# xubiker/deephisto

Measured on AMD Instinct MI355X. Metric: 256x256 patches/sec WSI inference (predict_full_patched), higher is better.
Workload: dtype bf16; 1 GPU; BASELINE configs[2]: predict_full_patched on one 50000x50000x3 closed-form synthetic WSI resident in HBM, 256x256 tiles stride 256, ResNet-18 (random init), bf16 MFMA, step = one whole slide (tile grid -> fused gather+forward -> all-gather -> ordered accumulate -> argmax); patch=256, stride=256, sampler_batch=64, micro_batch=4096, streams=1, downscale=16, n_tiles=38416, n_classes=5, parallelism=tile-range shard x1

## Files before the change

### deephisto_amd/_lib.py

```python
from __future__ import annotations

import ctypes as C
from pathlib import Path

import torch

LIB_PATH = Path(__file__).resolve().parent / "libdeephisto_hip.so"

DH_LAYOUT_NHWC, DH_LAYOUT_NCHW = 0, 1
DH_DTYPE_F32, DH_DTYPE_BF16 = 0, 1

_i32, _i64, _u32 = C.c_int32, C.c_int64, C.c_uint32
BUCKET_CB = C.CFUNCTYPE(None, C.c_int32, C.c_int64, C.c_int64, C.c_void_p)
_p = C.c_void_p

SIGNATURES = {
    "dh_abi_version": (C.c_int, []),
    "dh_last_error": (C.c_char_p, []),
    "dh_tile_grid_count": (C.c_int, [_i64, _i64, _i32, _i32, _i32, C.POINTER(_i64), C.POINTER(_i64)]),
    "dh_tile_grid": (C.c_int, [_i64, _i64, _i32, _i32, _i32, _p, _i64]),
    "dh_synth_slide": (C.c_int, [_p, _i64, _i64, _u32, _p]),
    "dh_tile_gather": (C.c_int, [_p, _i64, _i64, _p, _p, _i64, _i32, _i32, _i32, _p, _p]),
    "dh_tile_gather_aug": (C.c_int, [_p, _i64, _i64, _p, _i64, _i32, _i32, _i32, _i32, _i32, _p, _p]),
    "dh_tile_gather_stain_aug": (C.c_int, [_p, _i64, _i64, _p, _p, _p, _i64, _i32, _i32, _i32, _i32, _i32, _p, _p, _i32, _p, _i32, _p, _p]),
# ... 114 lines not shown
    "dh_debug_wgrad_bf16": (C.c_int, [_p, _p, _p] + [_i32] * 8 + [_p]),
    "dh_debug_conv_bf16": (C.c_int, [_p, _p, _p, _p] + [_i32] * 8 + [_p]),
    "dh_debug_conv_bn_act":(C.c_int, [_p, _p, _p, _p, _p, _p] + [_i32] * 9 + [_p]),
    "dh_debug_stem_out": (C.c_int, [_p, _i64, _i32, _p, _p]),
    "dh_debug_stem_pool_bf16": (C.c_int, [_p, _p, _i64, _i64, _p, _i64, _i32, _p, _p]),
    "dh_debug_wgrad_f32": (C.c_int, [_p, _p, _p] + [_i32] * 8 + [_p]),
    "dh_debug_stem_wgrad_f32": (C.c_int, [_p, _p, _p, _i32, _i32, _p]),
    "dh_debug_dgrad_f32": (C.c_int, [_p, _p, _p, _p] + [_i32] * 7 + [_p]),
    "dh_debug_pack_f32": (C.c_int, [_p, _i32, _i32, _p, _p, _p, _p, _p]),
    "dh_debug_pack_bf16": (C.c_int, [_p, _i32, _i32, _p, _p, _p, _p, _p]),
    "dh_debug_bn_f32": (C.c_int, [_p, _p, _p, _p, _i32, _p, _p, _p, _p, _p, _p, _p, _i64, _i32, _p]),
    "dh_debug_maxpool_f32": (C.c_int, [_p, _p, _p, _p, _i32, _i32, _i32, _i32, _p]),
    "dh_debug_bn_pool_f32": (C.c_int, [_p, _p, _p, _p, _p, _p, _p, _p, _p, _i32, _i32, _i32, _i32, _p]),
    "dh_debug_stamps": (C.c_int, [_i32, _p]),
    "dh_debug_stem_strip_width": (C.c_int, [_i32]),
    "dh_debug_last_conv3": (C.c_int, [_p, _p]),
    "dh_debug_env_knobs": (C.c_int, [C.c_char_p, _i64]),
    "dh_debug_coverage_set_map": (C.c_int, [_p, _p, _p]),
    "dh_debug_resnet18_forward_tap": (C.c_int, [_p, _p, _i64, _i64, _p, _i64, _i32, C.c_char_p, _p, _i32, _p, _i64, _p, _p]),
    "dh_debug_resnet50_forward_tap": (C.c_int, [_p, _p, _i64, _i64, _p, _i64, _i32, C.c_char_p, _p, _i32, _p, _i64, _p, _p]),
    "dh_debug_resnet18_operands": (C.c_int, [_p, C.c_char_p, _p, _i64, _p, _p, _i64]),
    "dh_debug_resnet50_operands": (C.c_int, [_p, C.c_char_p, _p, _i64, _p, _p, _i64]),
}


class DeephistoHipError(RuntimeError):
    pass


_lib = None
# ... 22 lines not shown
```

### deephisto_amd/csrc/conv3_tables_host.h

```cpp
#pragma once
#include <algorithm>
#include <array>
#include <cstdint>
#include <map>
#include <vector>

namespace dh_conv3 {

constexpr int kChunkBytes = 64;

struct TileDesc { int x, y, z, w; };

struct HostTables {
  std::vector<int> lane;
  std::vector<TileDesc> tile;
  std::vector<unsigned> mask;
  int grid = 0, threads = 0, lane_stride = 0, mask_rows = 0;
  bool xcd_group = false;
};

template <int STRIDE, int NT, int WAVES>
constexpr int max_window_pieces() { return (STRIDE == 2) ? (WAVES == 8 ? 5 : 10) : (NT == 2 ? 6 : 4); }

struct Cand { int th, tw, imgs, hp, variant, hr = 0, wtail = 0, fit = 0, ip = 0; };
// ... 154 lines not shown
inline int m16_read_conflicts(const int (&bl)[64]) {
  int extra = 0;
  for (int sg = 0; sg < 4; ++sg) {
    int cnt[16] = {0};
    for (int ll = 0; ll < 32; ++ll) {
      const bool in_a = ll < 4 || (ll >= 12 && ll < 16) || (ll >= 20 && ll < 28);
      if (in_a != ((sg & 1) == 0)) continue;
      const int l = (sg >> 1) * 32 + ll, G = l >> 4, slot = ((G & 1) << 1) | (G >> 1), w = bl[l];
      ++cnt[((w & 3) << 2) | (slot ^ ((w >> 2) & 3))];
    }
    for (int b = 0; b < 16; ++b) extra += cnt[b] > 1 ? cnt[b] - 1 : 0;
  }
  return extra;
}

template <int STRIDE, int NT, int WAVES, int ESZ, int MT, class P, bool HALF = false, bool M16 = false>
const char* build_tables(const P& p, int ncb, int grid_override, HostTables* out) {
  static_assert(!M16 || (STRIDE == 1 && !HALF && ESZ == 2), "M16: the stride-1 bf16 kernels");
  constexpr int MAXJ = max_window_pieces<STRIDE, NT, WAVES>();
  constexpr int NB = M16 ? 2 * NT : NT;
  const int threads = WAVES * 64, stride = 2 * NT + NB + MAXJ;
  constexpr int STAGE_PX_BYTES = HALF ? kChunkBytes / 2 : kChunkBytes;
  if ((int64_t)p.Cin * ESZ < 2 * STAGE_PX_BYTES || ((int64_t)p.Cin * ESZ) % STAGE_PX_BYTES) return "conv3x3: needs at least two whole channel stages per tile";
  const int64_t win_px = (int64_t)p.IMGS * p.HR * p.HP + p.WTAIL;
  const int IP = p.IP ? p.IP : p.HR * p.HP;
  if (win_px * STAGE_PX_BYTES > 65536) return "conv3x3: staged window larger than 64 KiB (16-bit fragment offsets)";
  if ((int64_t)p.n_win_instr * 1024 < win_px * STAGE_PX_BYTES) return "conv3x3: the DMA plan does not cover the staged window";
  constexpr int NTILE32 = (HALF ? WAVES / 2 : WAVES * MT / 2) * NT;
  if (p.FIT) {
    if (STRIDE != 1 || HALF) return "conv3x3: fit tiles are stride-1 tiles";
    if (p.IMGS * p.TH * p.TW > NTILE32 * 32) return "conv3x3: fit tile larger than the workgroup's slots";
    if (p.HP < p.TW + 1 || p.HR < p.TH + 1) return "conv3x3: fit tile pitch too small";
// ... 85 lines not shown
      for (int j = 0; j < MAXJ; ++j) {
        const auto& w = win[(size_t)tid * MAXJ + j];
        const int iy = oy0 * STRIDE + w[0] - 1, ix = ox0 * STRIDE + w[1] - 1;
        if (w[3] && w[2] < mk[2] && iy >= 0 && iy < p.Hi && ix >= 0 && ix < p.Wi) m |= 1u << j;
      }
      for (int nt = 0; nt < NT; ++nt) {
        const auto& q = pix[(size_t)tid * NT + nt];
        if (q[2] < mk[2] && oy0 + q[0] < p.Ho && ox0 + q[1] < p.Wo) m |= 1u << (16 + nt);
      }
      mask[(size_t)r * threads + tid] = m;
    }
    return r;
  };
  const int tiles_per_img = p.tiles_y * p.tiles_x;
  const int grid = grid_override > 0 ? grid_override : std::min(256, p.ntiles), n_pt = p.ntiles / ncb;
  const bool xcd_group = ncb > 1 && grid == 256 && 32 % ncb == 0 && (int64_t)p.Cout * p.Cin * 9 * ESZ <= (1 << 23);
  std::vector<TileDesc>& tile = out->tile;
  tile.assign((size_t)p.iters * grid, TileDesc{0, 0, 0, 0});
  for (int it = 0; it < p.iters; ++it)
    for (int w = 0; w < grid; ++w) {
      int cb, pt;
      if (xcd_group) {
        const int xcd = w % 8, slot = w / 8;
        cb = slot % ncb;
        pt = it * (grid / ncb) + (slot / ncb) * 8 + xcd;
      } else {
        const int T_ = it * grid + w;
        cb = T_ % ncb; pt = T_ / ncb;
      }
      const int valid = pt < n_pt ? 1 : 0, t = pt % tiles_per_img;
      const int img0 = valid ? (pt / tiles_per_img) * p.IMGS : 0, oy0 = (t / p.tiles_x) * p.TH, ox0 = (t % p.tiles_x) * p.TW;
      const int mrow = mask_row_of(img0, oy0, ox0);
      if (mrow >= 4096) return "conv3x3: too many distinct tile positions for the mask table";
      const int64_t win_off = (int64_t)img0 * img_in_bytes + ((int64_t)(oy0 * STRIDE) * p.Wi + ox0 * STRIDE) * p.in_px_bytes;
      const int64_t out_off = (int64_t)img0 * p.o_img + (int64_t)oy0 * p.o_row + (int64_t)ox0 * p.o_px + p.o_base + (int64_t)cb * p.out_cb;
      const int64_t res_off = (int64_t)img0 * p.o_img + (int64_t)oy0 * p.r_row + (int64_t)ox0 * p.r_px + p.r_base + (int64_t)cb * p.r_cb;
      if (win_off >= ((int64_t)1 << 32) || out_off >= ((int64_t)1 << 32) || res_off >= ((int64_t)1 << 32)) return "conv3x3: tensor larger than 4 Gi elements / bytes";
      const uint32_t word = (uint32_t)cb | (uint32_t)valid << 16 | (uint32_t)mrow << 20;
      tile[(size_t)it * grid + w] = TileDesc{(int)word, (int)(uint32_t)win_off, (int)(uint32_t)out_off, (int)(uint32_t)res_off};
    }
  out->grid = grid; out->threads = threads; out->lane_stride = stride; out->mask_rows = (int)mask_row.size(); out->xcd_group = xcd_group;
  return nullptr;
}

}
// ... 1 lines not shown
```

### deephisto_amd/csrc/env_knobs.h

```cpp
#pragma once

#define DH_ENV_KNOBS(X)                                                                                                                  \
  X(DH_CONV_S2_WIDE, 1, 0, 1, "load", "bf16 inference: 1 = wide stride-2 + downsample kernel (128 couts x 256 pixels), 0 = 128-pixel kernel")      \
  X(DH_CONV_FIT, 1, 0, 1, "load", "3x3 stride-1 convs on 7x7 / 14x14 maps: 1 = fit tiles (ten 7x7 images / five 7x14 half-images per 512 slots), 0 = power-of-two tiles")   \
  X(DH_CONV_MFMA16, 1, 0, 1, "load", "bf16 3x3 stride-1 convs: 1 = 16x16x32 MFMAs on the layers where they measured faster, 0 = 32x32x16 everywhere")   \
  X(DH_T1_SIDE, 1, 0, 1, "create", "float32 training engine: weight gradients on a low-priority side stream")                                     \
  X(DH_WGRAD3_WGS, 0, 0, 256, "load", "float32 3x3 weight gradient: workgroups per launch (0 = 224 with the side stream, else 256)")              \
  X(DH_T2_SIDE, 1, 0, 1, "create", "bf16 training engine: weight gradients, Adam and re-pack on a low-priority side stream")                       \
  X(DH_T2_JOIN, 1, 0, 1, "create", "bf16 engine: downsample branch's BN applied inside the join BN's pass (bit-identical either way)")            \
  X(DH_T2_FOLD, 1, 0, 1, "create", "bf16 engine: BN finalize folded into channel-sliced consumers on small maps (bit-identical either way)")      \
  X(DH_T2_FOLD_ROWS, 16384, 0, 1 << 24, "load", "bf16 engine: largest map (rows = B*H*W) that takes the folded BN path")                          \
  X(DH_G2_NSTAGE, 0, 0, 3, "load", "bf16 1x1 GEMM: LDS ring depth (0 = automatic: 2, or 3 from K >= DH_G2_NS3_K)")                                 \
  X(DH_G2_NS3_K, 512, 64, 1 << 20, "load", "bf16 1x1 GEMM: K from which the ring runs three stages deep")                                          \
  X(DH_G2_WIDE_M, 0, 0, 1 << 30, "load", "bf16 1x1 GEMM: 128 x 128 tiles for GEMMs of up to this many pixels (0 = off)")                          \
  X(DH_WGRAD_RING, 1, 0, 1, "load", "bf16 1x1 weight gradient: LDS-DMA ring kernel (0 = round-3 register-staged kernel)")                          \
  X(DH_WGRAD_RING_WGS, 0, 0, 1024, "load", "bf16 ring weight gradient: workgroups per launch (0 = 128 with the side stream, else 256)")           \
  X(DH_WGRAD2_WGS, 0, 0, 256, "load", "bf16 3x3 / 64-channel weight gradient: workgroups per launch (0 = 224 with the side stream, else 256)")
```

### deephisto_amd/csrc/resnet50_infer.inc

```

constexpr int R50_MAX_P = 256;
constexpr int64_t R50_MAX_TILES = ((int64_t)1 << 31) / ((int64_t)256 * (R50_MAX_P / 4) * (R50_MAX_P / 4) * 2);
static_assert(R50_MAX_TILES == DH_RESNET50_MAX_TILES, "include/deephisto_hip.h states the launch limit");

struct dh_resnet50 : InferNet {
  float* ones = nullptr;
  std::vector<int32_t> yx_host;
};

namespace {

struct R50GemmCfg { int nmt, nstage; };
R50GemmCfg r50_gemm_cfg(int N, int K) {
  R50GemmCfg c;
  c.nmt = (N % 128 == 0 && K <= 1024) ? 4 : 2;
  c.nstage = std::min(K / G2_BK, 2);
  return c;
}

int r50_gemm(const ConvLayer& L, const bf16_t* in, const bf16_t* res, bf16_t* out, int B, int Hi, int Wi, bool relu, hipStream_t st) {
  const int Ho = (Hi - 1) / L.stride + 1, Wo = (Wi - 1) / L.stride + 1;
  const int64_t M = (int64_t)B * Ho * Wo;
  DH_REQUIRE(L.ks == 1 && L.cout % 64 == 0 && L.cin % 64 == 0 && M > 0 && M < ((int64_t)1 << 31),
             "resnet50 1x1 %s: M=%lld N=%d K=%d unsupported", L.name.c_str(), (long long)M, L.cout, L.cin);
// ... 22 lines not shown
  auto al = [](size_t v) { return (v + 255) & ~(size_t)255; };
  const size_t px = (size_t)B * H2 * H2 * 2;
  const size_t big = al(256 * px), t1 = al(128 * px), t2 = al(64 * px);
  const size_t need = 2 * big + t1 + t2;
  int rc;
  if ((rc = infer_workspace(net, need))) return rc;
  char* base = static_cast<char*>(net->ws);
  bf16_t* X = reinterpret_cast<bf16_t*>(base);
  bf16_t* D = reinterpret_cast<bf16_t*>(base + big);
  bf16_t* T1 = reinterpret_cast<bf16_t*>(base + 2 * big);
  bf16_t* T2 = reinterpret_cast<bf16_t*>(base + 2 * big + t1);
  DH_REQUIRE(stem_seam_bytes(B, P) <= t1, "resnet50 forward: seam scratch larger than the bottleneck buffer");
  if ((rc = launch_stem_pool(net->convs[0], x, slide, slide_h, slide_w, yx, B, P, X, T1, st))) return rc;
  for (const char* nm : {"conv1", "maxpool"})
    if ((rc = tap_after<__bf16>(tap, nm, X, 64, H2, H2, 32, st))) return rc;
  int H = H2;
  for (const BlockDesc& b : net->desc->blocks) {
    const ConvLayer &c1 = net->convs[b.conv[0]], &c2 = net->convs[b.conv[1]], &c3 = net->convs[b.conv[2]];
    const int Ho = (H - 1) / b.stride + 1;
    if ((rc = r50_gemm(c1, X, nullptr, T1, B, H, H, true, st))) return rc;
    if ((rc = tap_after<__bf16>(tap, c1.name, T1, c1.cout, H, H, 32, st))) return rc;
    rc = b.stride == 1 ? launch_conv3x3<__bf16, 1>(c2, T1, nullptr, T2, B, H, H, true, st, Ho, Ho, nullptr, nullptr, true)
                       : launch_conv3x3<__bf16, 2>(c2, T1, nullptr, T2, B, H, H, true, st, Ho, Ho, nullptr, nullptr, true);
    if (rc) return rc;
    if ((rc = tap_after<__bf16>(tap, c2.name, T2, c2.cout, Ho, Ho, 32, st))) return rc;
    const bf16_t* idt = X;
    if (b.ds >= 0) {
      if ((rc = r50_gemm(net->convs[b.ds], X, nullptr, D, B, H, H, false, st))) return rc;
      if ((rc = tap_after<__bf16>(tap, net->convs[b.ds].name, D, c3.cout, Ho, Ho, 32, st))) return rc;
      idt = D;
    }
    if ((rc = r50_gemm(c3, T2, idt, X, B, Ho, Ho, true, st))) return rc;
    if ((rc = tap_after<__bf16>(tap, c3.name, X, c3.cout, Ho, Ho, 32, st))) return rc;
    H = Ho;
  }
  if (feat)
    hipLaunchKernelGGL(r50_head_kernel<true>, dim3(B), dim3(256), 0, st, X, H * H, net->fc_w_dev, net->fc_b_dev, net->n_classes, logits, feat);
  else if (logits)
// ... 133 lines not shown
```

### deephisto_amd/csrc/resnet_kernels.hip

```cpp
#include <math.h>
#include <stdlib.h>
#include <string.h>

#include <algorithm>
#include <array>
#include <atomic>
#include <map>
#include <mutex>
#include <set>
#include <string>
#include <vector>

#include "dh_common.h"
#include "conv3_tables_host.h"

typedef float f32x16 __attribute__((ext_vector_type(16)));
typedef float f32x4 __attribute__((ext_vector_type(4)));
typedef __bf16 bf16x8 __attribute__((ext_vector_type(8)));

namespace {

constexpr int CHUNK_BYTES = 64;
constexpr int PIX_PITCH = 80;
constexpr int FRAG_BYTES = 1024;
// ... 631 lines not shown
  if (it == g_zero_page.end()) {
    void* z = nullptr;
    DH_HIP(hipMalloc(&z, 1024));
    DH_HIP(hipMemset(z, 0, 1024));
    it = g_zero_page.emplace(dev, z).first;
  }
  *out = it->second;
  return DH_OK;
}

struct Conv3Tables { int* lane = nullptr; int4* tile = nullptr; unsigned* mask = nullptr; };
std::map<std::vector<int>, Conv3Tables> g_conv3_tables;
constexpr size_t CONV3_TABLE_CAP = 256;

template <int STRIDE, int NT, int WAVES, int ESZ, int MT, bool HALF = false, bool M16 = false>
int conv3_tables(const Conv3Params& p, int ncb, int groups_img, Conv3Tables* out, int grid_override = 0) {
  const std::vector<int> key = {current_device(), STRIDE, NT, WAVES, MT + (HALF ? 100 : 0) + (M16 ? 200 : 0), ESZ, p.TH, p.TW, p.IMGS, p.HR, p.HC, p.HP, p.HPH, p.Hi, p.Wi,
                                p.Cin, p.B, p.tiles_y, p.tiles_x, ncb, p.n_win_instr, p.WTAIL, p.FIT, p.IP, p.in_px_bytes, p.Ho, p.Wo, p.Cout, p.out_px,
                                p.out_cb, (int)(p.o_img & 0x7FFFFFFF), (int)(p.o_img >> 31), p.o_row, p.o_px, p.o_base, grid_override, p.iters,
                                p.r_row, p.r_px, p.r_cb, p.r_base};
  std::lock_guard<std::mutex> lk(g_host_mu);
  auto it = g_conv3_tables.find(key);
  if (it != g_conv3_tables.end()) { *out = it->second; return DH_OK; }
  if (g_conv3_tables.size() >= CONV3_TABLE_CAP) {
    for (auto& kv : g_conv3_tables) { (void)hipFree(kv.second.lane); (void)hipFree(kv.second.tile); (void)hipFree(kv.second.mask); }
    g_conv3_tables.clear();
  }
  dh_conv3::HostTables ht;
  if (const char* why = dh_conv3::build_tables<STRIDE, NT, WAVES, ESZ, MT, Conv3Params, HALF, M16>(p, ncb, grid_override, &ht)) { dh::set_error("%s", why); return DH_EINVAL; }
  static_assert(sizeof(dh_conv3::TileDesc) == sizeof(int4), "tile descriptor = int4");
  const std::vector<int>& lane = ht.lane;
  const std::vector<dh_conv3::TileDesc>& tile = ht.tile;
  const std::vector<unsigned>& mask = ht.mask;
  Conv3Tables tb;
  DH_HIP(hipMalloc((void**)&tb.lane, lane.size() * sizeof(int)));
  DH_HIP(hipMalloc((void**)&tb.tile, tile.size() * sizeof(int4)));
  DH_HIP(hipMalloc((void**)&tb.mask, mask.size() * sizeof(unsigned)));
  DH_HIP(hipMemcpy(tb.lane, lane.data(), lane.size() * sizeof(int), hipMemcpyHostToDevice));
  DH_HIP(hipMemcpy(tb.tile, tile.data(), tile.size() * sizeof(int4), hipMemcpyHostToDevice));
  DH_HIP(hipMemcpy(tb.mask, mask.data(), mask.size() * sizeof(unsigned), hipMemcpyHostToDevice));
  g_conv3_tables[key] = tb;
  *out = tb;
  (void)groups_img;
  return DH_OK;
}

template <typename T, int STRIDE, int NT, int WAVES, bool DS = false, int MT = 2, bool WRES = false, int CLS = -1, bool HALF = false, bool M16 = false>
int launch_conv3x3_cfg(Conv3Params& p, const ConvLayer& L, hipStream_t st) {
  constexpr int STAGE_PX_BYTES = HALF ? CHUNK_BYTES / 2 : CHUNK_BYTES, CO_BLK = HALF ? 128 : 64;
  const int win_px = p.IMGS * p.HR * p.HP + p.WTAIL;
  const int win_bytes = win_px * STAGE_PX_BYTES;
  const size_t wslab = (size_t)(9 + (DS ? 1 : 0)) * SLAB_TAP, win_alloc = (win_bytes + 1023) & ~1023;
  const size_t nchunks = (size_t)L.cin * sizeof(T) / STAGE_PX_BYTES;
  const size_t lds = (WRES ? nchunks * wslab + 2 * win_alloc : 2 * (wslab + win_alloc)) + (HALF ? 4096 : DS ? 2048 : 1024);

  constexpr int MAXJ = (STRIDE == 2) ? (WAVES == 8 ? 5 : 10) : (NT == 2 ? 6 : 4);
  p.n_win_instr = HALF ? (win_px + 31) / 32 : (win_px + 15) / 16;
  DH_REQUIRE(p.n_win_instr <= MAXJ * WAVES, "conv3x3: staging window too large for the DMA plan");
  DH_REQUIRE(lds <= 160 * 1024, "conv3x3: LDS budget exceeded (%zu B)", lds);
  DH_REQUIRE(p.FIT ? p.IMGS * p.TH * p.TW <= (WAVES * MT / 2) * NT * 32 && STRIDE == 1 && !HALF
                   : p.IMGS * p.TH * p.TW == (HALF ? WAVES / 2 : WAVES * MT / 2) * NT * 32, "conv3x3: tile/pixel mismatch");
  DH_REQUIRE(L.cin * (int)sizeof(T) >= 2 * CHUNK_BYTES, "conv3x3: needs at least two channel chunks");
  const int groups = ((p.B + p.IMGS - 1) / p.IMGS) * p.tiles_y * p.tiles_x;
  p.ntiles = groups * (L.cout / CO_BLK);
  const int grid = std::min(256, p.ntiles);
  DH_REQUIRE(!WRES || grid % (L.cout / 64) == 0, "conv3x3: resident weights need a fixed cout block per workgroup");
  p.iters = (p.ntiles + grid - 1) / grid;
  Conv3Tables tb;
  int rc = conv3_tables<STRIDE, NT, WAVES, (int)sizeof(T), MT, HALF, M16>(p, L.cout / CO_BLK, groups, &tb);
  if (rc) return rc;
  p.lane_tab = tb.lane; p.tile_tab = tb.tile; p.mask_tab = tb.mask;
  if constexpr (CLS >= 0) {
    if ((rc = ensure_dyn_lds(reinterpret_cast<const void*>(&conv3x3_kernel<T, STRIDE, NT, WAVES, false, DS, MT, WRES, CLS>), 160 * 1024))) return rc;
    hipLaunchKernelGGL((conv3x3_kernel<T, STRIDE, NT, WAVES, false, DS, MT, WRES, CLS>), dim3(grid), dim3(WAVES * 64), lds, st, p);
    DH_LAUNCH_CHECK();
    return DH_OK;
  }
  if ((rc = ensure_dyn_lds(reinterpret_cast<const void*>(&conv3x3_kernel<T, STRIDE, NT, WAVES, false, DS, MT, WRES, -1, HALF, M16>), 160 * 1024)) ||
      (rc = ensure_dyn_lds(reinterpret_cast<const void*>(&conv3x3_kernel<T, STRIDE, NT, WAVES, true, DS, MT, WRES, -1, HALF, M16>), 160 * 1024))) return rc;
  if (p.stamps) hipLaunchKernelGGL((conv3x3_kernel<T, STRIDE, NT, WAVES, true, DS, MT, WRES, -1, HALF, M16>), dim3(grid), dim3(WAVES * 64), lds, st, p);
  else hipLaunchKernelGGL((conv3x3_kernel<T, STRIDE, NT, WAVES, false, DS, MT, WRES, -1, HALF, M16>), dim3(grid), dim3(WAVES * 64), lds, st, p);
  DH_LAUNCH_CHECK();
  return DH_OK;
}

inline bool s2_wide_eligible(const ConvLayer& c1, const ConvLayer& ds, int esz, int Wo) {
  static const bool on = dh::env_int("DH_CONV_S2_WIDE") != 0;
  return on && esz == 2 && c1.w2_dev && ds.w2_dev && c1.cout % 128 == 0 && Wo > 4;
}

inline bool conv3_mfma16_layer(int cin, int cout) {
  static const bool on = dh::env_int("DH_CONV_MFMA16") != 0;
  return DH_CONV_HOIST && on && cin == cout && (cin == 64 || cin == 256 || cin == 512);
}
std::atomic<int> g_last_conv3_variant{-1}, g_last_conv3_mfma{0};

template <typename T, int STRIDE, int CLS = -1>
int launch_conv3x3(const ConvLayer& L, const void* in, const void* res, void* out, int B, int Hi, int Wi,
                   bool relu, hipStream_t st, int Ho, int Wo, const ConvLayer* ds = nullptr, void* ds_out = nullptr,
                   bool blocked = false, int full_h = 0, int full_w = 0, bool in16 = false, bool out16 = false) {
  Conv3Params p;
  static_assert(CLS < 0 || STRIDE == 1, "parity classes run on the stride-1 kernel");
  DH_REQUIRE(blocked || (!in16 && !out16), "conv3x3: 16-channel planes are a variant of the channel-blocked layout");
  DH_REQUIRE(CLS < 0 || (!blocked && !ds && full_h > 0 && full_w > 0), "conv3x3: a parity class needs the NHWC layout and the size of dX");
  DH_REQUIRE(!blocked || sizeof(T) == 2, "conv3x3: the channel-blocked layout is the bf16 inference layout");
  if (blocked) {
    p.in_px_bytes = CHUNK_BYTES; p.in_chunk_bytes = Hi * Wi * CHUNK_BYTES;
    p.out_px = 32; p.out_mt = Ho * Wo * 32; p.out_cb = 2 * p.out_mt;
  } else {
    p.in_px_bytes = L.cin * (int)sizeof(T); p.in_chunk_bytes = CHUNK_BYTES;
    p.out_px = L.cout; p.out_mt = 32; p.out_cb = 64;
  }
  if (CLS >= 0) {
    p.o_img = (int64_t)full_h * full_w * L.cout; p.o_row = 2 * full_w * L.cout; p.o_px = 2 * L.cout;
    p.o_base = ((CLS >> 1) * full_w + (CLS & 1)) * L.cout;
  } else {
// ... 43 lines not shown
    g_last_conv3_variant = -1; g_last_conv3_mfma = 32;
    if constexpr (CLS >= 0)
      rc = variant == 0 ? launch_conv3x3_cfg<T, 1, 2, 8, false, 2, false, CLS>(p, L, st)
         : variant == 1 ? launch_conv3x3_cfg<T, 1, 1, 8, false, 2, false, CLS>(p, L, st)
                        : launch_conv3x3_cfg<T, 1, 1, 8, false, 1, false, CLS>(p, L, st);
    else {
      constexpr bool BF16 = sizeof(T) == 2;
      const bool wres = BF16 && variant == 0 && wres_lds <= 160 * 1024;
      bool m16 = false;
#if DH_CONV_HOIST
      if constexpr (BF16) m16 = conv3_mfma16_layer(L.cin, L.cout);
#endif
      g_last_conv3_variant = variant; g_last_conv3_mfma = m16 ? 16 : 32;
      if constexpr (BF16 && DH_CONV_HOIST) {
        if (m16)
          rc = wres         ? launch_conv3x3_cfg<T, 1, 2, 8, false, 2, true, -1, false, true>(p, L, st)
             : variant == 0 ? launch_conv3x3_cfg<T, 1, 2, 8, false, 2, false, -1, false, true>(p, L, st)
             : variant == 1 ? launch_conv3x3_cfg<T, 1, 1, 8, false, 2, false, -1, false, true>(p, L, st)
                            : launch_conv3x3_cfg<T, 1, 1, 8, false, 1, false, -1, false, true>(p, L, st);
      }
      if (!m16)
        rc = wres         ? launch_conv3x3_cfg<T, 1, 2, 8, false, 2, BF16>(p, L, st)
           : variant == 0 ? launch_conv3x3_cfg<T, 1, 2, 8>(p, L, st)
           : variant == 1 ? launch_conv3x3_cfg<T, 1, 1, 8>(p, L, st)
                          : launch_conv3x3_cfg<T, 1, 1, 8, false, 1>(p, L, st);
    }
  } else {
    g_last_conv3_variant = -1; g_last_conv3_mfma = 32;
    static const bool s2_wide = dh::env_int("DH_CONV_S2_WIDE") != 0;
    if constexpr (sizeof(T) == 2) {
      if (in16) {
        DH_REQUIRE(s2_wide && ds && blocked && L.w2_dev && ds->w2_dev && L.cout % 128 == 0 && dh_conv3::set_stride2_wide_geometry(p, Ho, Wo),
                   "conv3x3: an input in 16-channel planes needs the wide stride-2 kernel");
        p.w = L.w2_dev; p.ds_w = ds->w2_dev;
        p.out_cb = 4 * p.out_mt;
        return launch_conv3x3_cfg<T, 2, 2, 8, true, 2, false, -1, true>(p, L, st);
      }
    }
    dh_conv3::set_stride2_geometry(p, Ho, Wo);
    const size_t wres_lds = (size_t)L.cin * sizeof(T) / CHUNK_BYTES * (ds ? 10 : 9) * SLAB_TAP
                          + 2 * (((size_t)p.IMGS * p.HR * p.HP * CHUNK_BYTES + 1023) & ~(size_t)1023) + 2048;
    if (ds && sizeof(T) == 2 && wres_lds <= 160 * 1024) rc = launch_conv3x3_cfg<T, 2, 1, 8, true, 1, true>(p, L, st);
    else rc = ds ? launch_conv3x3_cfg<T, 2, 1, 8, true, 1>(p, L, st) : launch_conv3x3_cfg<T, 2, 1, 8, false, 1>(p, L, st);
  }
  if (rc) return rc;
  if (sample) {
    DH_HIP(hipEventRecord(g_prof.ev[g_prof.used + 1], st));
    g_prof.used += 2;
    g_prof.flops += 2.0 * B * Ho * Wo * (double)L.cout * 9 * L.cin;
  }
  return DH_OK;
}

template <typename T, int NT, int WAVES, int MT>
int launch_dgrad_s2_merged_cfg(Conv3Params (&pc)[4], const int (&tiles_c)[4], const ConvLayer& L, hipStream_t st) {
  static const int order[4] = {3, 1, 2, 0}, taps[4] = {4, 2, 2, 1};
  constexpr int MAXJ = NT == 2 ? 6 : 4;
  const Conv3Params& p0 = pc[0];
// ... 110 lines not shown
    p.in = dz; p.w = L.w_dev; p.scale = L.scale_dev; p.shift = L.shift_dev; p.res = res; p.out = dx;
    p.B = B; p.Hi = Ho; p.Wi = Wo; p.Cin = L.cin; p.Cout = L.cout; p.Ho = rows; p.Wo = cols;
    p.relu = 0; p.zero_page = zp; p.stamps = nullptr;
    p.HPH = 0; p.TH = cd.th; p.TW = cd.tw; p.IMGS = cd.imgs; p.HP = cd.hp; p.HR = cd.th + 2; p.HC = cd.tw + 2;
    p.tiles_y = (rows + cd.th - 1) / cd.th; p.tiles_x = (cols + cd.tw - 1) / cd.tw;
    p.lane_tab = nullptr; p.tile_tab = nullptr; p.mask_tab = nullptr; p.ntiles = 0; p.iters = 0; p.n_win_instr = 0;
    tiles_c[k] = tiles_of(cd, rows, cols);
  }
  return cd.variant == 0 ? launch_dgrad_s2_merged_cfg<T, 2, 8, 2>(pc, tiles_c, L, st)
       : cd.variant == 1 ? launch_dgrad_s2_merged_cfg<T, 1, 8, 2>(pc, tiles_c, L, st)
                         : launch_dgrad_s2_merged_cfg<T, 1, 8, 1>(pc, tiles_c, L, st);
}

template <typename T>
int run_conv(const ConvLayer& L, const void* in, const void* res, void* out, int B, int Hi, int Wi,
             bool relu, hipStream_t st, int* Ho_out, int* Wo_out, bool blocked = false, bool out16 = false) {
  const int pad = L.ks / 2;
  const int Ho = (Hi + 2 * pad - L.ks) / L.stride + 1, Wo = (Wi + 2 * pad - L.ks) / L.stride + 1;
  *Ho_out = Ho; *Wo_out = Wo;
  DH_REQUIRE((int64_t)B * Hi * Wi * L.cin * (int64_t)sizeof(T) < ((int64_t)1 << 32),
             "conv %s: input larger than 4 GiB, reduce the batch", L.name.c_str());
  if (L.ks == 3 && L.stride == 1) return launch_conv3x3<T, 1>(L, in, res, out, B, Hi, Wi, relu, st, Ho, Wo, nullptr, nullptr, blocked, 0, 0, false, out16);
  DH_REQUIRE(!out16, "conv %s: only the stride-1 3x3 kernel writes 16-channel planes", L.name.c_str());
  if (L.ks == 3 && L.stride == 2) return launch_conv3x3<T, 2>(L, in, res, out, B, Hi, Wi, relu, st, Ho, Wo, nullptr, nullptr, blocked);
  DH_REQUIRE(!blocked, "conv %s: only the 3x3 kernels read the channel-blocked layout", L.name.c_str());
  ConvParams p;
  p.in = in; p.w = L.w_dev; p.scale = L.scale_dev; p.shift = L.shift_dev; p.res = res; p.out = out;
  p.B = B; p.Hi = Hi; p.Wi = Wi; p.Cin = L.cin; p.Cout = L.cout; p.Ho = Ho; p.Wo = Wo;
  if (p.Ho > 8 || p.Wo > 8) { p.TH = 16; p.TW = 16; p.IMGS = 1; }
  else { p.TH = 8; p.TW = 8; p.IMGS = 4; }
  p.tiles_y = (p.Ho + p.TH - 1) / p.TH; p.tiles_x = (p.Wo + p.TW - 1) / p.TW;
  p.relu = relu ? 1 : 0;
  if (L.ks == 1 && L.stride == 2) return launch_conv<T, 1, 2, false>(p, st);
  dh::set_error("conv %s: unsupported shape", L.name.c_str());
  return DH_EINVAL;
}

int g_stem_pc_force = 0;

// ... 118 lines not shown
  }
  {
    const int64_t total = (int64_t)B * H2 * H2 * (64 / (16 / esz));
    const int grid = (int)std::min<int64_t>((total + 255) / 256, 256 * 32);
    hipLaunchKernelGGL((maxpool_kernel<T>), dim3(grid), dim3(256), 0, st, static_cast<const T*>(S),
                       static_cast<T*>(bufA), B, H1, H1, 64, H2, H2);
    DH_LAUNCH_CHECK();
    if (int rc = tap_after<T>(tap, "maxpool", bufA, 64, H2, H2, 64, st)) return rc;
  }
  }
  constexpr bool BLK = sizeof(T) == 2;
  int H = H2, W = H2;
  bool x16 = false;
  void* X = bufA;
  const std::vector<BlockDesc>& blocks = net->desc->blocks;
  for (size_t bi = 0; bi < blocks.size(); ++bi) {
    const BlockDesc& b = blocks[bi];
    const bool has_ds = b.ds >= 0;
    const ConvLayer& c1 = net->convs[b.conv[0]];
    const ConvLayer& c2 = net->convs[b.conv[1]];
    void* other = X == bufA ? bufC : bufA;
    int Ho, Wo, h2, w2;
    int rc;
    const void* resid = X;
    if (has_ds) {
      Ho = (H + 2 - 3) / 2 + 1; Wo = (W + 2 - 3) / 2 + 1;
      rc = launch_conv3x3<T, 2>(c1, X, nullptr, bufB, B, H, W, true, st, Ho, Wo, &net->convs[b.ds], other, BLK, 0, 0, x16, false);
      if (rc) return rc;
      if ((rc = tap_after<T>(tap, net->convs[b.ds].name, other, c1.cout, Ho, Wo, BLK ? 32 : c1.cout, st))) return rc;
      resid = other;
    } else {
      DH_REQUIRE(!x16, "resnet18 forward: only a downsample block reads 16-channel planes");
      rc = run_conv<T>(c1, X, nullptr, bufB, B, H, W, true, st, &Ho, &Wo, BLK);
      if (rc) return rc;
    }
    if ((rc = tap_after<T>(tap, c1.name, bufB, c1.cout, Ho, Wo, BLK ? 32 : c1.cout, st))) return rc;
    x16 = false;
    if (bi + 1 < blocks.size() && blocks[bi + 1].stride == 2) {
      const BlockDesc& nb = blocks[bi + 1];
      x16 = BLK && s2_wide_eligible(net->convs[nb.conv[0]], net->convs[nb.ds], esz, (Wo + 2 - 3) / 2 + 1);
    }
    void* O = X;
    if (has_ds) O = X;
    else if (x16) O = other;
    rc = run_conv<T>(c2, bufB, resid, O, B, Ho, Wo, true, st, &h2, &w2, BLK, x16);
    if (rc) return rc;
    if ((rc = tap_after<T>(tap, c2.name, O, c2.cout, Ho, Wo, x16 ? 16 : BLK ? 32 : c2.cout, st))) return rc;
    X = O;
    H = Ho; W = Wo;
  }
  if (feat)
    hipLaunchKernelGGL((avgpool_fc_kernel<T, true>), dim3(B), dim3(256), 0, st, static_cast<const T*>(X), H * W,
                       net->desc->feat, BLK ? 1 : 0, net->fc_w_dev, net->fc_b_dev, net->n_classes, logits, feat);
  else if (logits)
    hipLaunchKernelGGL((avgpool_fc_kernel<T, false>), dim3(B), dim3(256), 0, st, static_cast<const T*>(X), H * W,
                       net->desc->feat, BLK ? 1 : 0, net->fc_w_dev, net->fc_b_dev, net->n_classes, logits, nullptr);
  DH_LAUNCH_CHECK();
  if (cam) return launch_cam_head<T>(net, X, B, H * W, cam, st);
  return DH_OK;
}
// ... 231 lines not shown
  if (out64_host) {
    if (!g_stamps_dev) { memset(out64_host, 0, 64 * sizeof(unsigned long long)); return DH_OK; }
    DH_HIP(hipDeviceSynchronize());
    DH_HIP(hipMemcpy(out64_host, g_stamps_dev, 64 * sizeof(unsigned long long), hipMemcpyDeviceToHost));
    DH_HIP(hipMemset(g_stamps_dev, 0, 64 * sizeof(unsigned long long)));
  }
  return DH_OK;
}

extern "C" int dh_debug_last_conv3(int32_t* variant, int32_t* mfma_m) {
  DH_REQUIRE(variant && mfma_m, "dh_debug_last_conv3: null argument");
  *variant = g_last_conv3_variant; *mfma_m = g_last_conv3_mfma;
  return DH_OK;
}

extern "C" int dh_debug_stem_strip_width(int32_t pc) {
  DH_REQUIRE(pc == 0 || pc == 15 || pc == 16, "debug stem strip width: %d is not 0, 15 or 16", pc);
  g_stem_pc_force = pc;
  return DH_OK;
}

#include "gemm1x1_f32.inc"
#include "train_core.inc"
#include "train.inc"
#include "train2_kernels.inc"
#include "wgrad_ring.inc"
#include "bn_fold.inc"
#include "gemm1x1.inc"
#include "train2.inc"
#include "train_hooks.inc"
// ... 3 lines not shown
```

### include/deephisto_hip_debug.h

```cpp
#ifndef DEEPHISTO_HIP_DEBUG_H
#define DEEPHISTO_HIP_DEBUG_H

#include "deephisto_hip.h"

#ifdef __cplusplus
extern "C" {
#endif

int dh_train2_debug_act(dh_train2* net, const char* conv_name, int32_t what, float* out_dev, int64_t n_elem, void* stream);
int dh_resnet18_train_debug_act(dh_resnet18* net, const char* conv_name, int32_t what, float* out_dev, int64_t n_elem, void* stream);

int dh_train2_debug_backward_tap(dh_train2* net, const float* dlogits_dev, const char* conv_name, float* grad_in_dev, int64_t n_elem,
                                 float* g_out_dev, float* mean_dev, float* invstd_dev, int32_t* route_host, void* stream);

int dh_debug_pack_bf16(const float* w_dev, int32_t cout, int32_t cin, uint16_t* wf_tile, uint16_t* wd_tile, uint16_t* wf_elem,
                       uint16_t* wd_elem, void* stream);
int dh_debug_gemm1x1_bf16(const uint16_t* a_dev, const uint16_t* w_dev, const uint16_t* res_dev, uint16_t* out_dev, int64_t M,
                          int32_t N, int32_t K, int32_t stride, int32_t Ho, int32_t Wo, int32_t Hi, int32_t Wi, int32_t repeat,
                          void* stream);
int dh_debug_gemm1x1_fused_bf16(const uint16_t* a_dev, const uint16_t* w_dev, const uint16_t* res_dev, const uint16_t* mask_dev,
                                uint16_t* out_dev, float* mean_dev, float* invstd_dev, int64_t M, int32_t N, int32_t K, int32_t stride,
                                int32_t Ho, int32_t Wo, int32_t Hi, int32_t Wi, int32_t repeat, void* stream);
int dh_debug_gemm1x1_bwdsums_bf16(const uint16_t* a_dev, const uint16_t* w_dev, const uint16_t* res_dev, const uint16_t* mask_dev,
                                  uint16_t* out_dev, const uint16_t* z_dev, const float* mean_dev, const float* invstd_dev,
// ... 38 lines not shown
                       int32_t cin, int32_t cout, int32_t ks, int32_t stride, int32_t mode, void* stream);
int dh_debug_stem_wgrad_f32(const float* dz_dev, const float* x_nchw_dev, float* dw_dev, int32_t B, int32_t P, void* stream);
int dh_debug_dgrad_f32(const float* dz_dev, const float* w_dev, const float* res_dev, float* dx_dev, int32_t B, int32_t Hi,
                       int32_t Wi, int32_t cin, int32_t cout, int32_t ks, int32_t stride, void* stream);
int dh_debug_pack_f32(const float* w_dev, int32_t cout, int32_t cin, float* wf_tile, float* wd_tile, float* wf_elem, float* wd_elem,
                      void* stream);
int dh_debug_bn_f32(const float* z_dev, const float* gamma_dev, const float* beta_dev, const float* res_dev, int32_t relu,
                    float* y_dev, const float* dy_dev, float* dz_dev, float* g_dev, float* dgamma_dev, float* dbeta_dev,
                    float* stats_out_dev, int64_t rows, int32_t C, void* stream);
int dh_debug_maxpool_f32(const float* x_dev, float* y_dev, const float* dy_dev, float* dx_dev, int32_t B, int32_t Hi, int32_t Wi,
                         int32_t C, void* stream);
int dh_debug_bn_pool_f32(const float* z_dev, const float* gamma_dev, const float* beta_dev, float* pooled_dev, uint8_t* idx_dev,
                         const float* dpool_dev, float* dz_dev, float* dgamma_dev, float* dbeta_dev, int32_t B, int32_t Hi, int32_t Wi,
                         int32_t C, void* stream);
int dh_debug_stem_strip_width(int32_t pooled_columns);
int dh_debug_stamps(int32_t enable, unsigned long long* out64_host);
int dh_debug_last_conv3(int32_t* variant, int32_t* mfma_m);
int dh_debug_env_knobs(char* buf_host, int64_t cap);

int dh_debug_resnet18_forward_tap(dh_resnet18* net, const uint8_t* slide, int64_t h, int64_t w, const int32_t* yx_dev, int64_t n, int32_t P,
                                  const char* conv_name, const int32_t* sel_dev, int32_t k, float* out_dev, int64_t out_elems,
                                  float* logits_dev, void* stream);
int dh_debug_resnet50_forward_tap(dh_resnet50* net, const uint8_t* slide, int64_t h, int64_t w, const int32_t* yx_dev, int64_t n, int32_t P,
                                  const char* conv_name, const int32_t* sel_dev, int32_t k, float* out_dev, int64_t out_elems,
                                  float* logits_dev, void* stream);
int dh_debug_resnet18_operands(dh_resnet18* net, const char* conv_name, float* w_host, int64_t w_elems, float* scale_host,
                               float* shift_host, int64_t c_elems);
int dh_debug_resnet50_operands(dh_resnet50* net, const char* conv_name, float* w_host, int64_t w_elems, float* scale_host,
                               float* shift_host, int64_t c_elems);

// ... 7 lines not shown
```

Before: 226,100 patches/s.

## Add per-layer conv3x3 tile schedules: image-local XCD grouping and alternating reverse order

Adds new tile-to-workgroup schedule policies to the 3x3 conv table builder. One keeps each XCD on a contiguous run of images, aimed at L2 locality of activations. The other reverses the tile order on every second launch so the next layer starts on tiles whose inputs are still hot in cache. By default (mode 0), the channel-blocked ResNet-18 path picks a policy per layer class: reverse order on even positions, plus image-local grouping for the 64-channel layers. It also adds an env knob and a debug override, at the cost of more cached table variants and possible worse balance across XCDs.

New measurement: 227,700 patches/s, median of 6. No clear change (+0.7%).

```diff
diff --git a/deephisto_amd/_lib.py b/deephisto_amd/_lib.py
--- a/deephisto_amd/_lib.py
+++ b/deephisto_amd/_lib.py
@@ -152,6 +152,7 @@
     "dh_debug_bn_pool_f32": (C.c_int, [_p, _p, _p, _p, _p, _p, _p, _p, _p, _i32, _i32, _i32, _i32, _p]),
     "dh_debug_stamps": (C.c_int, [_i32, _p]),
     "dh_debug_stem_strip_width": (C.c_int, [_i32]),
+    "dh_debug_conv_sched": (C.c_int, [_i32]),
     "dh_debug_last_conv3": (C.c_int, [_p, _p]),
     "dh_debug_env_knobs": (C.c_int, [C.c_char_p, _i64]),
     "dh_debug_coverage_set_map": (C.c_int, [_p, _p, _p]),
diff --git a/deephisto_amd/csrc/conv3_tables_host.h b/deephisto_amd/csrc/conv3_tables_host.h
--- a/deephisto_amd/csrc/conv3_tables_host.h
+++ b/deephisto_amd/csrc/conv3_tables_host.h
@@ -192,8 +192,31 @@
   return extra;
 }
 
+enum : int { kSchedLegacy = 0, kSchedImageLocal = 1, kSchedReverse = 2 };
+struct SchedSlot { int cb, pt, valid; };
+inline bool sched_xcd_group(int grid, int ncb, int64_t weight_bytes) { return ncb > 1 && grid == 256 && 32 % ncb == 0 && weight_bytes <= (1 << 23); }
+inline bool sched_image_local_applies(int grid, int ncb, bool xcd_group) { return grid == 256 && ncb >= 1 && 32 % ncb == 0 && (ncb == 1 || xcd_group); }
+inline SchedSlot schedule_slot(int policy, int it, int w, int grid, int ncb, int n_pt, bool xcd_group) {
+  SchedSlot s;
+  if ((policy & kSchedImageLocal) && sched_image_local_applies(grid, ncb, xcd_group)) {
+    const int xcd = w % 8, slot = w / 8, run = 32 / ncb;
+    s.cb = slot % ncb;
+    s.pt = it * (grid / ncb) + xcd * run + slot / ncb;
+  } else if (xcd_group) {
+    const int xcd = w % 8, slot = w / 8;
+    s.cb = slot % ncb;
+    s.pt = it * (grid / ncb) + (slot / ncb) * 8 + xcd;
+  } else {
+    const int T_ = it * grid + w;
+    s.cb = T_ % ncb; s.pt = T_ / ncb;
+  }
+  s.valid = s.pt < n_pt ? 1 : 0;
+  if ((policy & kSchedReverse) && s.valid) s.pt = n_pt - 1 - s.pt;
+  return s;
+}
+
 template <int STRIDE, int NT, int WAVES, int ESZ, int MT, class P, bool HALF = false, bool M16 = false>
-const char* build_tables(const P& p, int ncb, int grid_override, HostTables* out) {
+const char* build_tables(const P& p, int ncb, int grid_override, HostTables* out, int policy = kSchedLegacy) {
   static_assert(!M16 || (STRIDE == 1 && !HALF && ESZ == 2), "M16: the stride-1 bf16 kernels");
   constexpr int MAXJ = max_window_pieces<STRIDE, NT, WAVES>();
   constexpr int NB = M16 ? 2 * NT : NT;
@@ -309,21 +332,14 @@
   };
   const int tiles_per_img = p.tiles_y * p.tiles_x;
   const int grid = grid_override > 0 ? grid_override : std::min(256, p.ntiles), n_pt = p.ntiles / ncb;
-  const bool xcd_group = ncb > 1 && grid == 256 && 32 % ncb == 0 && (int64_t)p.Cout * p.Cin * 9 * ESZ <= (1 << 23);
+  const bool xcd_group = sched_xcd_group(grid, ncb, (int64_t)p.Cout * p.Cin * 9 * ESZ);
   std::vector<TileDesc>& tile = out->tile;
   tile.assign((size_t)p.iters * grid, TileDesc{0, 0, 0, 0});
   for (int it = 0; it < p.iters; ++it)
     for (int w = 0; w < grid; ++w) {
-      int cb, pt;
-      if (xcd_group) {
-        const int xcd = w % 8, slot = w / 8;
-        cb = slot % ncb;
-        pt = it * (grid / ncb) + (slot / ncb) * 8 + xcd;
-      } else {
-        const int T_ = it * grid + w;
-        cb = T_ % ncb; pt = T_ / ncb;
-      }
-      const int valid = pt < n_pt ? 1 : 0, t = pt % tiles_per_img;
+      const SchedSlot sl = schedule_slot(policy, it, w, grid, ncb, n_pt, xcd_group);
+      const int cb = sl.cb, pt = sl.pt;
+      const int valid = sl.valid, t = pt % tiles_per_img;
       const int img0 = valid ? (pt / tiles_per_img) * p.IMGS : 0, oy0 = (t / p.tiles_x) * p.TH, ox0 = (t % p.tiles_x) * p.TW;
       const int mrow = mask_row_of(img0, oy0, ox0);
       if (mrow >= 4096) return "conv3x3: too many distinct tile positions for the mask table";
diff --git a/deephisto_amd/csrc/env_knobs.h b/deephisto_amd/csrc/env_knobs.h
--- a/deephisto_amd/csrc/env_knobs.h
+++ b/deephisto_amd/csrc/env_knobs.h
@@ -4,6 +4,7 @@
   X(DH_CONV_S2_WIDE, 1, 0, 1, "load", "bf16 inference: 1 = wide stride-2 + downsample kernel (128 couts x 256 pixels), 0 = 128-pixel kernel")      \
   X(DH_CONV_FIT, 1, 0, 1, "load", "3x3 stride-1 convs on 7x7 / 14x14 maps: 1 = fit tiles (ten 7x7 images / five 7x14 half-images per 512 slots), 0 = power-of-two tiles")   \
   X(DH_CONV_MFMA16, 1, 0, 1, "load", "bf16 3x3 stride-1 convs: 1 = 16x16x32 MFMAs on the layers where they measured faster, 0 = 32x32x16 everywhere")   \
+  X(DH_CONV_SCHED, 0, 0, 4, "load", "bf16 inference 3x3 convs, tile schedule: 0 = per layer class, 1 = legacy everywhere, 2 = image-local XCDs, 3 = every second launch back to front, 4 = both")   \
   X(DH_T1_SIDE, 1, 0, 1, "create", "float32 training engine: weight gradients on a low-priority side stream")                                     \
   X(DH_WGRAD3_WGS, 0, 0, 256, "load", "float32 3x3 weight gradient: workgroups per launch (0 = 224 with the side stream, else 256)")              \
   X(DH_T2_SIDE, 1, 0, 1, "create", "bf16 training engine: weight gradients, Adam and re-pack on a low-priority side stream")                       \
diff --git a/deephisto_amd/csrc/resnet50_infer.inc b/deephisto_amd/csrc/resnet50_infer.inc
--- a/deephisto_amd/csrc/resnet50_infer.inc
+++ b/deephisto_amd/csrc/resnet50_infer.inc
@@ -60,14 +60,15 @@
   if ((rc = launch_stem_pool(net->convs[0], x, slide, slide_h, slide_w, yx, B, P, X, T1, st))) return rc;
   for (const char* nm : {"conv1", "maxpool"})
     if ((rc = tap_after<__bf16>(tap, nm, X, 64, H2, H2, 32, st))) return rc;
-  int H = H2;
+  int H = H2, pos3 = 0;
   for (const BlockDesc& b : net->desc->blocks) {
     const ConvLayer &c1 = net->convs[b.conv[0]], &c2 = net->convs[b.conv[1]], &c3 = net->convs[b.conv[2]];
     const int Ho = (H - 1) / b.stride + 1;
     if ((rc = r50_gemm(c1, X, nullptr, T1, B, H, H, true, st))) return rc;
     if ((rc = tap_after<__bf16>(tap, c1.name, T1, c1.cout, H, H, 32, st))) return rc;
-    rc = b.stride == 1 ? launch_conv3x3<__bf16, 1>(c2, T1, nullptr, T2, B, H, H, true, st, Ho, Ho, nullptr, nullptr, true)
-                       : launch_conv3x3<__bf16, 2>(c2, T1, nullptr, T2, B, H, H, true, st, Ho, Ho, nullptr, nullptr, true);
+    rc = b.stride == 1 ? launch_conv3x3<__bf16, 1>(c2, T1, nullptr, T2, B, H, H, true, st, Ho, Ho, nullptr, nullptr, true, 0, 0, false, false, Conv3SchedAt{pos3, false})
+                       : launch_conv3x3<__bf16, 2>(c2, T1, nullptr, T2, B, H, H, true, st, Ho, Ho, nullptr, nullptr, true, 0, 0, false, false, Conv3SchedAt{pos3, false});
+    ++pos3;
     if (rc) return rc;
     if ((rc = tap_after<__bf16>(tap, c2.name, T2, c2.cout, Ho, Ho, 32, st))) return rc;
     const bf16_t* idt = X;
diff --git a/deephisto_amd/csrc/resnet_kernels.hip b/deephisto_amd/csrc/resnet_kernels.hip
--- a/deephisto_amd/csrc/resnet_kernels.hip
+++ b/deephisto_amd/csrc/resnet_kernels.hip
@@ -669,11 +669,11 @@
 constexpr size_t CONV3_TABLE_CAP = 256;
 
 template <int STRIDE, int NT, int WAVES, int ESZ, int MT, bool HALF = false, bool M16 = false>
-int conv3_tables(const Conv3Params& p, int ncb, int groups_img, Conv3Tables* out, int grid_override = 0) {
+int conv3_tables(const Conv3Params& p, int ncb, int groups_img, Conv3Tables* out, int grid_override = 0, int sched = dh_conv3::kSchedLegacy) {
   const std::vector<int> key = {current_device(), STRIDE, NT, WAVES, MT + (HALF ? 100 : 0) + (M16 ? 200 : 0), ESZ, p.TH, p.TW, p.IMGS, p.HR, p.HC, p.HP, p.HPH, p.Hi, p.Wi,
                                 p.Cin, p.B, p.tiles_y, p.tiles_x, ncb, p.n_win_instr, p.WTAIL, p.FIT, p.IP, p.in_px_bytes, p.Ho, p.Wo, p.Cout, p.out_px,
                                 p.out_cb, (int)(p.o_img & 0x7FFFFFFF), (int)(p.o_img >> 31), p.o_row, p.o_px, p.o_base, grid_override, p.iters,
-                                p.r_row, p.r_px, p.r_cb, p.r_base};
+                                p.r_row, p.r_px, p.r_cb, p.r_base, sched};
   std::lock_guard<std::mutex> lk(g_host_mu);
   auto it = g_conv3_tables.find(key);
   if (it != g_conv3_tables.end()) { *out = it->second; return DH_OK; }
@@ -682,7 +682,7 @@
     g_conv3_tables.clear();
   }
   dh_conv3::HostTables ht;
-  if (const char* why = dh_conv3::build_tables<STRIDE, NT, WAVES, ESZ, MT, Conv3Params, HALF, M16>(p, ncb, grid_override, &ht)) { dh::set_error("%s", why); return DH_EINVAL; }
+  if (const char* why = dh_conv3::build_tables<STRIDE, NT, WAVES, ESZ, MT, Conv3Params, HALF, M16>(p, ncb, grid_override, &ht, sched)) { dh::set_error("%s", why); return DH_EINVAL; }
   static_assert(sizeof(dh_conv3::TileDesc) == sizeof(int4), "tile descriptor = int4");
   const std::vector<int>& lane = ht.lane;
   const std::vector<dh_conv3::TileDesc>& tile = ht.tile;
@@ -701,7 +701,7 @@
 }
 
 template <typename T, int STRIDE, int NT, int WAVES, bool DS = false, int MT = 2, bool WRES = false, int CLS = -1, bool HALF = false, bool M16 = false>
-int launch_conv3x3_cfg(Conv3Params& p, const ConvLayer& L, hipStream_t st) {
+int launch_conv3x3_cfg(Conv3Params& p, const ConvLayer& L, hipStream_t st, int sched = dh_conv3::kSchedLegacy) {
   constexpr int STAGE_PX_BYTES = HALF ? CHUNK_BYTES / 2 : CHUNK_BYTES, CO_BLK = HALF ? 128 : 64;
   const int win_px = p.IMGS * p.HR * p.HP + p.WTAIL;
   const int win_bytes = win_px * STAGE_PX_BYTES;
@@ -722,7 +722,7 @@
   DH_REQUIRE(!WRES || grid % (L.cout / 64) == 0, "conv3x3: resident weights need a fixed cout block per workgroup");
   p.iters = (p.ntiles + grid - 1) / grid;
   Conv3Tables tb;
-  int rc = conv3_tables<STRIDE, NT, WAVES, (int)sizeof(T), MT, HALF, M16>(p, L.cout / CO_BLK, groups, &tb);
+  int rc = conv3_tables<STRIDE, NT, WAVES, (int)sizeof(T), MT, HALF, M16>(p, L.cout / CO_BLK, groups, &tb, 0, sched);
   if (rc) return rc;
   p.lane_tab = tb.lane; p.tile_tab = tb.tile; p.mask_tab = tb.mask;
   if constexpr (CLS >= 0) {
@@ -748,13 +748,31 @@
   static const bool on = dh::env_int("DH_CONV_MFMA16") != 0;
   return DH_CONV_HOIST && on && cin == cout && (cin == 64 || cin == 256 || cin == 512);
 }
+struct Conv3SchedAt { int pos = -1; bool by_class = false; };
+int g_conv3_sched_force = 0;
+inline int conv3_sched_class(int stride, int cin, int cout, bool residual) {
+  const bool local = cin == 64 && ((stride == 1 && cout == 64 && residual) || (stride == 2 && cout == 128));
+  return dh_conv3::kSchedReverse | (local ? dh_conv3::kSchedImageLocal : dh_conv3::kSchedLegacy);
+}
+inline int conv3_sched(int stride, int cin, int cout, bool residual, Conv3SchedAt at) {
+  static const int env = dh::env_int("DH_CONV_SCHED");
+  if (at.pos < 0) return dh_conv3::kSchedLegacy;
+  const int mode = g_conv3_sched_force ? g_conv3_sched_force : env;
+  const int bits = mode == 0 ? (at.by_class ? conv3_sched_class(stride, cin, cout, residual) : dh_conv3::kSchedLegacy)
+                 : mode == 1 ? dh_conv3::kSchedLegacy
+                 : mode == 2 ? dh_conv3::kSchedImageLocal
+                 : mode == 3 ? dh_conv3::kSchedReverse
+                             : dh_conv3::kSchedImageLocal | dh_conv3::kSchedReverse;
+  return at.pos % 2 == 0 ? bits : bits & ~dh_conv3::kSchedReverse;
+}
 std::atomic<int> g_last_conv3_variant{-1}, g_last_conv3_mfma{0};
 
 template <typename T, int STRIDE, int CLS = -1>
 int launch_conv3x3(const ConvLayer& L, const void* in, const void* res, void* out, int B, int Hi, int Wi,
                    bool relu, hipStream_t st, int Ho, int Wo, const ConvLayer* ds = nullptr, void* ds_out = nullptr,
-                   bool blocked = false, int full_h = 0, int full_w = 0, bool in16 = false, bool out16 = false) {
+                   bool blocked = false, int full_h = 0, int full_w = 0, bool in16 = false, bool out16 = false, Conv3SchedAt sched_at = {}) {
   Conv3Params p;
+  const int sched = CLS < 0 ? conv3_sched(STRIDE, L.cin, L.cout, res != nullptr, sched_at) : dh_conv3::kSchedLegacy;
   static_assert(CLS < 0 || STRIDE == 1, "parity classes run on the stride-1 kernel");
   DH_REQUIRE(blocked || (!in16 && !out16), "conv3x3: 16-channel planes are a variant of the channel-blocked layout");
   DH_REQUIRE(CLS < 0 || (!blocked && !ds && full_h > 0 && full_w > 0), "conv3x3: a parity class needs the NHWC layout and the size of dX");
@@ -828,16 +846,16 @@
       g_last_conv3_variant = variant; g_last_conv3_mfma = m16 ? 16 : 32;
       if constexpr (BF16 && DH_CONV_HOIST) {
         if (m16)
-          rc = wres         ? launch_conv3x3_cfg<T, 1, 2, 8, false, 2, true, -1, false, true>(p, L, st)
-             : variant == 0 ? launch_conv3x3_cfg<T, 1, 2, 8, false, 2, false, -1, false, true>(p, L, st)
-             : variant == 1 ? launch_conv3x3_cfg<T, 1, 1, 8, false, 2, false, -1, false, true>(p, L, st)
-                            : launch_conv3x3_cfg<T, 1, 1, 8, false, 1, false, -1, false, true>(p, L, st);
+          rc = wres         ? launch_conv3x3_cfg<T, 1, 2, 8, false, 2, true, -1, false, true>(p, L, st, sched)
+             : variant == 0 ? launch_conv3x3_cfg<T, 1, 2, 8, false, 2, false, -1, false, true>(p, L, st, sched)
+             : variant == 1 ? launch_conv3x3_cfg<T, 1, 1, 8, false, 2, false, -1, false, true>(p, L, st, sched)
+                            : launch_conv3x3_cfg<T, 1, 1, 8, false, 1, false, -1, false, true>(p, L, st, sched);
       }
       if (!m16)
-        rc = wres         ? launch_conv3x3_cfg<T, 1, 2, 8, false, 2, BF16>(p, L, st)
-           : variant == 0 ? launch_conv3x3_cfg<T, 1, 2, 8>(p, L, st)
-           : variant == 1 ? launch_conv3x3_cfg<T, 1, 1, 8>(p, L, st)
-                          : launch_conv3x3_cfg<T, 1, 1, 8, false, 1>(p, L, st);
+        rc = wres         ? launch_conv3x3_cfg<T, 1, 2, 8, false, 2, BF16>(p, L, st, sched)
+           : variant == 0 ? launch_conv3x3_cfg<T, 1, 2, 8>(p, L, st, sched)
+           : variant == 1 ? launch_conv3x3_cfg<T, 1, 1, 8>(p, L, st, sched)
+                          : launch_conv3x3_cfg<T, 1, 1, 8, false, 1>(p, L, st, sched);
     }
   } else {
     g_last_conv3_variant = -1; g_last_conv3_mfma = 32;
@@ -848,14 +866,14 @@
                    "conv3x3: an input in 16-channel planes needs the wide stride-2 kernel");
         p.w = L.w2_dev; p.ds_w = ds->w2_dev;
         p.out_cb = 4 * p.out_mt;
-        return launch_conv3x3_cfg<T, 2, 2, 8, true, 2, false, -1, true>(p, L, st);
+        return launch_conv3x3_cfg<T, 2, 2, 8, true, 2, false, -1, true>(p, L, st, sched);
       }
     }
     dh_conv3::set_stride2_geometry(p, Ho, Wo);
     const size_t wres_lds = (size_t)L.cin * sizeof(T) / CHUNK_BYTES * (ds ? 10 : 9) * SLAB_TAP
                           + 2 * (((size_t)p.IMGS * p.HR * p.HP * CHUNK_BYTES + 1023) & ~(size_t)1023) + 2048;
-    if (ds && sizeof(T) == 2 && wres_lds <= 160 * 1024) rc = launch_conv3x3_cfg<T, 2, 1, 8, true, 1, true>(p, L, st);
-    else rc = ds ? launch_conv3x3_cfg<T, 2, 1, 8, true, 1>(p, L, st) : launch_conv3x3_cfg<T, 2, 1, 8, false, 1>(p, L, st);
+    if (ds && sizeof(T) == 2 && wres_lds <= 160 * 1024) rc = launch_conv3x3_cfg<T, 2, 1, 8, true, 1, true>(p, L, st, sched);
+    else rc = ds ? launch_conv3x3_cfg<T, 2, 1, 8, true, 1>(p, L, st, sched) : launch_conv3x3_cfg<T, 2, 1, 8, false, 1>(p, L, st, sched);
   }
   if (rc) return rc;
   if (sample) {
@@ -996,15 +1014,15 @@
 
 template <typename T>
 int run_conv(const ConvLayer& L, const void* in, const void* res, void* out, int B, int Hi, int Wi,
-             bool relu, hipStream_t st, int* Ho_out, int* Wo_out, bool blocked = false, bool out16 = false) {
+             bool relu, hipStream_t st, int* Ho_out, int* Wo_out, bool blocked = false, bool out16 = false, Conv3SchedAt sched_at = {}) {
   const int pad = L.ks / 2;
   const int Ho = (Hi + 2 * pad - L.ks) / L.stride + 1, Wo = (Wi + 2 * pad - L.ks) / L.stride + 1;
   *Ho_out = Ho; *Wo_out = Wo;
   DH_REQUIRE((int64_t)B * Hi * Wi * L.cin * (int64_t)sizeof(T) < ((int64_t)1 << 32),
              "conv %s: input larger than 4 GiB, reduce the batch", L.name.c_str());
-  if (L.ks == 3 && L.stride == 1) return launch_conv3x3<T, 1>(L, in, res, out, B, Hi, Wi, relu, st, Ho, Wo, nullptr, nullptr, blocked, 0, 0, false, out16);
+  if (L.ks == 3 && L.stride == 1) return launch_conv3x3<T, 1>(L, in, res, out, B, Hi, Wi, relu, st, Ho, Wo, nullptr, nullptr, blocked, 0, 0, false, out16, sched_at);
   DH_REQUIRE(!out16, "conv %s: only the stride-1 3x3 kernel writes 16-channel planes", L.name.c_str());
-  if (L.ks == 3 && L.stride == 2) return launch_conv3x3<T, 2>(L, in, res, out, B, Hi, Wi, relu, st, Ho, Wo, nullptr, nullptr, blocked);
+  if (L.ks == 3 && L.stride == 2) return launch_conv3x3<T, 2>(L, in, res, out, B, Hi, Wi, relu, st, Ho, Wo, nullptr, nullptr, blocked, 0, 0, false, false, sched_at);
   DH_REQUIRE(!blocked, "conv %s: only the 3x3 kernels read the channel-blocked layout", L.name.c_str());
   ConvParams p;
   p.in = in; p.w = L.w_dev; p.scale = L.scale_dev; p.shift = L.shift_dev; p.res = res; p.out = out;
@@ -1153,6 +1171,8 @@
   bool x16 = false;
   void* X = bufA;
   const std::vector<BlockDesc>& blocks = net->desc->blocks;
+  int pos3 = 0;
+  auto next_pos = [&]() { return BLK ? Conv3SchedAt{pos3++, true} : Conv3SchedAt{}; };
   for (size_t bi = 0; bi < blocks.size(); ++bi) {
     const BlockDesc& b = blocks[bi];
     const bool has_ds = b.ds >= 0;
@@ -1164,13 +1184,13 @@
     const void* resid = X;
     if (has_ds) {
       Ho = (H + 2 - 3) / 2 + 1; Wo = (W + 2 - 3) / 2 + 1;
-      rc = launch_conv3x3<T, 2>(c1, X, nullptr, bufB, B, H, W, true, st, Ho, Wo, &net->convs[b.ds], other, BLK, 0, 0, x16, false);
+      rc = launch_conv3x3<T, 2>(c1, X, nullptr, bufB, B, H, W, true, st, Ho, Wo, &net->convs[b.ds], other, BLK, 0, 0, x16, false, next_pos());
       if (rc) return rc;
       if ((rc = tap_after<T>(tap, net->convs[b.ds].name, other, c1.cout, Ho, Wo, BLK ? 32 : c1.cout, st))) return rc;
       resid = other;
     } else {
       DH_REQUIRE(!x16, "resnet18 forward: only a downsample block reads 16-channel planes");
-      rc = run_conv<T>(c1, X, nullptr, bufB, B, H, W, true, st, &Ho, &Wo, BLK);
+      rc = run_conv<T>(c1, X, nullptr, bufB, B, H, W, true, st, &Ho, &Wo, BLK, false, next_pos());
       if (rc) return rc;
     }
     if ((rc = tap_after<T>(tap, c1.name, bufB, c1.cout, Ho, Wo, BLK ? 32 : c1.cout, st))) return rc;
@@ -1182,7 +1202,7 @@
     void* O = X;
     if (has_ds) O = X;
     else if (x16) O = other;
-    rc = run_conv<T>(c2, bufB, resid, O, B, Ho, Wo, true, st, &h2, &w2, BLK, x16);
+    rc = run_conv<T>(c2, bufB, resid, O, B, Ho, Wo, true, st, &h2, &w2, BLK, x16, next_pos());
     if (rc) return rc;
     if ((rc = tap_after<T>(tap, c2.name, O, c2.cout, Ho, Wo, x16 ? 16 : BLK ? 32 : c2.cout, st))) return rc;
     X = O;
@@ -1444,6 +1464,12 @@
   return DH_OK;
 }
 
+extern "C" int dh_debug_conv_sched(int32_t mode) {
+  DH_REQUIRE(mode >= 0 && mode <= 4, "debug conv schedule: mode %d is not 0 .. 4", mode);
+  g_conv3_sched_force = mode;
+  return DH_OK;
+}
+
 extern "C" int dh_debug_stem_strip_width(int32_t pc) {
   DH_REQUIRE(pc == 0 || pc == 15 || pc == 16, "debug stem strip width: %d is not 0, 15 or 16", pc);
   g_stem_pc_force = pc;
diff --git a/include/deephisto_hip_debug.h b/include/deephisto_hip_debug.h
--- a/include/deephisto_hip_debug.h
+++ b/include/deephisto_hip_debug.h
@@ -76,6 +76,7 @@
                          const float* dpool_dev, float* dz_dev, float* dgamma_dev, float* dbeta_dev, int32_t B, int32_t Hi, int32_t Wi,
                          int32_t C, void* stream);
 int dh_debug_stem_strip_width(int32_t pooled_columns);
+int dh_debug_conv_sched(int32_t mode);
 int dh_debug_stamps(int32_t enable, unsigned long long* out64_host);
 int dh_debug_last_conv3(int32_t* variant, int32_t* mfma_m);
 int dh_debug_env_knobs(char* buf_host, int64_t cap);
```
